# jiexray/gelly-streaming

Hardware: AMD Instinct MI355X
Metric: edges/sec (whole node) for streaming CC on RMAT-26 (higher is better)
Workload: dtype int64; 1 GPU; rmat26-cc-stream; scale=26, edges=1073741824, micro_batch=1048576, combine_every_edges_per_gpu=4194304, combine=none at 1 GPU (same cadence), ids=sparse 64-bit (scrambled), capacity_hint=33554432, vertices_labelled=32802821, parallelism=single GPU

## Files before the change

### gelly-streaming_amd/__init__.py

```python
import ctypes
import os

import numpy as np


_HERE = os.path.dirname(os.path.abspath(__file__))
LIB_PATH = os.path.join(_HERE, "lib", "libgs_summary.so")
if os.environ.get("GS_LIB_VARIANT"):
    LIB_PATH = os.path.join(_HERE, "lib_" + os.environ["GS_LIB_VARIANT"], "libgs_summary.so")

KIND_CC = 0
KIND_SIGNED = 1
KIND_DEGREE = 2

DEGREE_ALL = 0
DEGREE_IN = 1
DEGREE_OUT = 2

GS_OK = 0
GS_ERR_INVALID = -1
GS_ERR_HIP = -2
GS_ERR_CAPACITY = -3
GS_ERR_TRUNCATED = -4
GS_ERR_PARSE = -5
# ... 442 lines not shown


def digest_rows(v, label, parity=None):
    import torch

    def srl(x, k):
        return (x >> k) & ((1 << (64 - k)) - 1)

    def mix(z):
        z = (z ^ srl(z, 30)) * -4658895280553007687
        z = (z ^ srl(z, 27)) * -7723592293110705685
        return z ^ srl(z, 31)
    if v.numel() == 0:
        return 0
    a = mix(v ^ 0x243F6A8885A308D3)
    b = mix(label + (parity.to(torch.int64) * 0x13198A2E03707344 if parity is not None else 0))
    return int(torch.sum(a * b).item()) & ((1 << 64) - 1)


TESTING_KNOBS = {"server_idle_us": 0, "changes_walk_max": 1, "parse_lb_timeout_us": 2, "group_self_apply": 3,
                 "group_data_lag": 4, "degree_variant": 5, "triangle_variant": 6, "triangle_profile": 7,
                 "slice_profile": 8, "distinct_profile": 9, "spanner_round_cap": 10, "spanner_lds_set": 11,
                 "spanner_arenas": 12}


def testing_set(knob, value):
    _check(lib().gs_testing_set(TESTING_KNOBS[knob], -1 if value is None else int(value)))


def testing_get(knob):
    return lib().gs_testing_get(TESTING_KNOBS[knob])


def testing_hot_tune(summary, rows=None, sketch_log2=None, sample_folds=None):
    for what, v in enumerate((rows, sketch_log2, sample_folds)):
        if v is not None:
            _check(lib().gs_testing_hot_tune(summary._h, what, int(v)))


def testing_hot_keys(summary):
    import numpy as np
    n = lib().gs_testing_hot_keys(summary._h, None, 0)
    if n < 0:
        _check(int(n))
    out = (_i64 * max(int(n), 1))()
    m = lib().gs_testing_hot_keys(summary._h, out, int(n))
    if m < 0:
        _check(int(m))
    return np.frombuffer(out, dtype=np.int64, count=int(min(n, m))).copy()


class testing:

    def __init__(self, **knobs):
        self.knobs = knobs

    def __enter__(self):
        for k, v in self.knobs.items():
            testing_set(k, v)
        return self

    def __exit__(self, *a):
        for k in self.knobs:
            testing_set(k, None)


FAKE_COMM_PATH = os.path.join(_HERE, "host", "bin", "libgs_fakecomm.so")
_fake = None
# ... 1609 lines not shown
```

### gelly-streaming_amd/csrc/gs_capi.cpp

```cpp
#include <hip/hip_runtime.h>

#include <algorithm>
#include <atomic>
#include <chrono>
#include <mutex>
#include <unordered_map>
#include <cstdio>
#include <cstring>
#include <string>
#include <thread>
#include <vector>

#include "gs_ingest.h"
#include "gs_internal.hpp"

#ifndef GS_YOUNG_HEAD_LOG2
#define GS_YOUNG_HEAD_LOG2 14
#endif

namespace gsi {

thread_local std::string g_err;

int fail(int code, const std::string& msg) {
// ... 574 lines not shown

int fold_device_impl(gs_summary* h, const int64_t* src, const int64_t* dst, const uint8_t* w, size_t n,
                     size_t stride, size_t w_stride, bool track, bool check_cap, const FoldSource& fs) {
  if (n == 0) return GS_OK;
  const uint64_t units = fs.rows ? fs.units : n;
  if (track && !fs.take_out) {
    uint64_t fill = h->delta_fill_ub[h->dset];
    for (size_t off = 0; off < n; off += kMaxChunk) fill += per_shard_edges(std::min<size_t>(kMaxChunk, n - off));
    if (!h->drec || fill > h->delta_shard_cap)
      return fail(GS_ERR_CAPACITY, "delta list full: stage or take the delta records after at most " +
                                       std::to_string(h->delta_edges) + " folded edges");
  }
  constexpr int young_head_log2 = GS_YOUNG_HEAD_LOG2;
  const bool young_head = young_head_log2 > 0 && check_cap && !track && !fs.take_out && fs.lane < 0 && !fs.on_side &&
                          h->e_launched == 0 && h->nv_exact == 0 && n > ((size_t)2 << young_head_log2);
  if (check_cap && units) {
    if (int rc = ensure_capacity(h, units)) return rc;
  }
  const bool pipe = fs.allow_pipe && h->pipe_depth > 1 && (!track || fs.pipe_tracked) && fs.rows == 0 &&
                    !h->profiling && !h->changes;
  const bool on_lane = fs.lane >= 0 && !h->profiling;
  const bool side = fs.on_side && side_ok(h) && !track;
  if (!pipe && !side && !on_lane) {
    if (int rc = join_pipe_lanes(h)) return rc;
  }
  const bool sign = h->kind == GS_KIND_SIGNED;
  const int hot = (check_cap && !track && !fs.take_out && fs.rows == 0 && !fs.on_side && fs.lane < 0 && !fs.n_dev &&
                   stride != 3)
                      ? hot_log2(h)
                      : 0;
  for (size_t off = 0, c = 0; off < n; off += c) {
    const bool head = young_head && off == 0;
    c = head ? ((size_t)1 << young_head_log2) : std::min<size_t>(kMaxChunk, n - off);
    const uint32_t blocks = (uint32_t)((c + gs::kFoldBS - 1) / gs::kFoldBS);
    if (track && !fs.take_out) h->delta_fill_ub[h->dset] += per_shard_edges(c);
    hipStream_t st = side ? h->side : h->stream;
    if (side) h->side_dirty = true;
    if (head) {
      if (int rc = join_pipe_lanes(h)) return rc;
    } else if (pipe) {
      st = h->lane[h->lane_next];
      h->last_lane = h->lane_next;
      h->lane_next = (h->lane_next + 1) % h->pipe_depth;
      GS_HIP(hipEventRecord(h->main_ev, h->stream));
      if (hipEventQuery(h->main_ev) != hipSuccess) GS_HIP(hipStreamWaitEvent(st, h->main_ev, 0));
      h->lanes_dirty = true;
    } else if (on_lane) {
      st = h->lane[fs.lane];
      h->last_lane = fs.lane;
      h->lanes_dirty = true;
    }
    gs::FoldLaunch f;
    f.src = src + off * stride;
    f.dst = dst + off * stride;
    f.w = w ? w + off * w_stride : nullptr;
    f.n = c;
    f.stride = (uint32_t)stride;
    f.w_stride = (uint32_t)w_stride;
    if (h->dedup && !w && stride == 1 && fs.rows == 0 && !fs.n_dev) {
      int set = 0;
      if (st == h->side) set = gs_summary::kDedupSets - 1;
      for (int li = 0; li < gs_summary::kLanes; ++li)
        if (st == h->lane[li]) set = 1 + li;
      if (h->dd_edges[set] < c) {
        GS_HIP(hipStreamSynchronize(st));
        h->dd_edges[set] = 0;
        const uint64_t e = next_pow2(c);
        GS_HIP(h->dd_tab[set].alloc(2 * e * 2));
        GS_HIP(h->dd_w[set].alloc(e));
        h->dd_edges[set] = e;
      }
      const uint64_t slots = 2 * next_pow2(c);
      GS_HIP(hipMemsetAsync(h->dd_tab[set], 0xFF, slots * 16, st));
      GS_LAUNCH(gs::launch_dedup(f.src, f.dst, c, h->dd_tab[set], (uint32_t)(slots - 1), h->dd_w[set], st));
      f.w = h->dd_w[set];
      f.w_stride = 1;
    }
    f.rows = fs.rows;
    f.skip_rank = fs.skip_rank;
    f.counts = fs.counts;
    f.base = (uint32_t)off;
    f.n_dev = fs.n_dev;
    f.fail_in = off == 0 ? fs.fail_in : nullptr;
    f.shard0 = h->shard0;
    if (fs.take_out) {
      f.take_out = fs.take_out;
      f.take_cap = fs.take_cap;
      f.take_count = fs.take_count;
      f.done = h->done_dev;
      f.seq = *fs.take_seq = ++h->done_seq;
    }
    h->shard0 = (h->shard0 + blocks) & (gs::kShards - 1);
    const int rs = report_stream(h, st);
    const bool carry = check_cap && units && !fs.take_out && !fs.n_dev && h->rep_pending[rs];
    if (carry) {
      f.rep_out = h->rep.dev() + (h->rep_seq++ % gs_summary::kRepRing);
      f.rep_claim = h->rep_pending[rs];
      f.rep_epoch = (unsigned)(h->rep_epoch & 7u);
    }
    if (hot) {
      if (int rc = hot_before_fold(h)) return rc;
      if (h->hot_live >= 0 && h->hot_alloc_log2 == hot) {
        f.hot.e = h->hot_buf[h->hot_live];
        f.hot.shift = 65 - hot;
      }
    }
    {
      Prof p(h, KID_FOLD, st);
      gs::launch_fold(sign, track, h->table(), h->delta(), f, st);
    }
    GS_HIP(hipGetLastError());
    if (carry) {
      h->rep_pending_edges -= f.rep_claim;
      h->rep_pending[rs] = 0;
    }
    if (check_cap && units) {
      const uint64_t cu = fs.rows ? (off + c >= n ? units : 0) : c;
      h->rep_pending[rs] += cu;
      h->rep_pending_edges += cu;
      if (fs.n_dev && !fs.take_out)
        if (int rc = launch_report_now(h, rs, st)) return rc;
    }
    if (hot)
      if (int rc = hot_after_fold(h, f.src, f.dst, c, stride, st, hot)) return rc;
  }
  return GS_OK;
}

int join_into_last_lane(gs_summary* h, hipStream_t* es, bool* on_lane) {
  if (int rc = server_stop(h)) return rc;
  *es = h->stream;
  *on_lane = h->lanes_dirty && !h->side_dirty && h->last_lane >= 0 && h->lane[h->last_lane] && !h->profiling;
  if (!*on_lane) return join_lanes(h);
  *es = h->lane[h->last_lane];
  for (int i = 0; i < gs_summary::kLanes && h->lane[i]; ++i) {
    if (i == h->last_lane) continue;
    GS_HIP(hipEventRecord(h->lane[i].ev, h->lane[i]));
    GS_HIP(hipStreamWaitEvent(*es, h->lane[i].ev, 0));
  }
  GS_HIP(hipEventRecord(h->main_ev, h->stream));
  if (h->xwait || hipEventQuery(h->main_ev) != hipSuccess) GS_HIP(hipStreamWaitEvent(*es, h->main_ev, 0));
  return GS_OK;
// ... 1070 lines not shown
    h->hot_alloc_log2 = 0;
    for (auto& b : h->hot_buf) b.reset();
    h->hot_scratch.reset();
  }
  h->hot_cfg = log2_entries < 0 ? -1 : log2_entries;
  h->hot_first = first_after_edges;
  h->hot_every = rebuild_every_folds;
  return GS_OK;
}

int gs_hot_index_stats(gs_handle h, uint64_t* out4) {
  if (int rc = check_any(h)) return rc;
  if (!out4) return fail(GS_ERR_INVALID, "out is null");
  DeviceGuard g(h->device);
  if (int rc = join_lanes(h)) return rc;
  GS_HIP(hipStreamSynchronize(h->stream));
  if (int rc = hot_before_fold(h)) return rc;
  out4[0] = h->hot_builds;
  out4[1] = 0;
  out4[2] = h->hot_live >= 0 ? (uint64_t)h->hot_alloc_log2 : 0;
  out4[3] = h->hot_refreshes;
  if (h->hot_live >= 0) {
    std::vector<gs::HotBucket> e(gs::hot_buckets(h->hot_alloc_log2));
    GS_HIP(hipMemcpy(e.data(), h->hot_buf[h->hot_live], e.size() * sizeof(gs::HotBucket), hipMemcpyDeviceToHost));
    for (const gs::HotBucket& x : e) out4[1] += (x.key[0] != gs::kEmpty) + (x.key[1] != gs::kEmpty);
  }
  return GS_OK;
}

int gs_testing_hot_tune(void* hv, int what, int64_t value) {
  gs_handle h = static_cast<gs_handle>(hv);
  if (int rc = check_any(h)) return rc;
  if (h->kind != GS_KIND_CC) return fail(GS_ERR_INVALID, "the hot index serves connected-components summaries only");
  if (what < 0 || what > 2) return fail(GS_ERR_INVALID, "hot tune: what is 0, 1 or 2");
  if (value >= 0) {
    if (what == 0 && value != 1 && value != 2) return fail(GS_ERR_INVALID, "hot tune: 1 or 2 sketch rows");
    if (what == 1 && value > 6) return fail(GS_ERR_INVALID, "hot tune: at most 2^6 counters per id");
    if (what == 2 && value != 1 && value != 2 && value != 4) return fail(GS_ERR_INVALID, "hot tune: 1, 2 or 4 sample folds");
  }
  DeviceGuard g(h->device);
  if (int rc = join_lanes(h)) return rc;
  GS_HIP(hipStreamSynchronize(h->stream));
  hot_drop(h);
  h->hot_alloc_log2 = 0;
  for (auto& b : h->hot_buf) b.reset();
  h->hot_scratch.reset();
  if (what == 0) h->hot_rows = value < 0 ? 0 : (int)value;
  if (what == 1) h->hot_sketch_log2 = value < 0 ? -1 : (int)value;
  if (what == 2) h->hot_sample_folds = value < 0 ? 0u : (uint32_t)value;
  return GS_OK;
}

int64_t gs_testing_hot_keys(void* hv, int64_t* out, uint64_t cap) {
  gs_handle h = static_cast<gs_handle>(hv);
  if (int rc = check_any(h)) return rc;
  if (!out && cap) return fail(GS_ERR_INVALID, "out is null");
  DeviceGuard g(h->device);
  if (int rc = join_lanes(h)) return rc;
  GS_HIP(hipStreamSynchronize(h->stream));
  if (int rc = hot_before_fold(h)) return rc;
  if (h->hot_live < 0) return 0;
  std::vector<gs::HotBucket> e(gs::hot_buckets(h->hot_alloc_log2));
  GS_HIP(hipMemcpy(e.data(), h->hot_buf[h->hot_live], e.size() * sizeof(gs::HotBucket), hipMemcpyDeviceToHost));
  uint64_t n = 0;
  for (const gs::HotBucket& x : e)
    for (int64_t k : x.key)
      if (k != gs::kEmpty) {
// ... 58 lines not shown
```

### gelly-streaming_amd/csrc/gs_internal.hpp

```cpp
#pragma once
#include <hip/hip_runtime.h>

#include <string>
#include <vector>

#include "gs_devbuf.hpp"
#include "gs_grow.hpp"
#include "gs_hostio.hpp"
#include "gs_ingest.hpp"
#include "gs_kernels.hpp"
#include "gs_own.hpp"
#include "gs_sort.hpp"
#include "gs_summary.h"
#include "gs_testing.h"

namespace gsi {

int fail(int code, const std::string& msg);
int64_t testing_value(int knob, int64_t product);

constexpr int kMaxDevices = 64;
uint64_t create_capacity(uint64_t capacity_hint);
uint64_t create_bytes(uint64_t cap);

// ... 274 lines not shown
  uint64_t deg_total = 0;
  gsi::TextIngest text;
  int pipe_depth = 1;
  uint64_t api_calls = 0;
  int group_lanes = 0;
  static constexpr int kLanes = 4;
  gsi::Lane lane[kLanes];
  gsi::Event main_ev;
  gsi::Event idle_ev;
  bool xwait = false;
  int lane_next = 0;
  int last_lane = -1;
  bool lanes_dirty = false;
  bool export_ctr_zero = false;
  int hot_cfg = 0;
  uint64_t hot_first = 0;
  uint32_t hot_every = 0;
  gsi::DevBuf<gs::HotBucket> hot_buf[2];
  gsi::DevBuf<unsigned long long> hot_scratch;
  int hot_alloc_log2 = 0;
  int hot_live = -1;
  int hot_building = -1;
  gsi::Event hot_built;
  gsi::Event hot_read[2][kLanes + 1];
  bool hot_read_on[2] = {false, false};
  uint64_t hot_edges = 0;
  uint32_t hot_folds = 0;
  uint32_t hot_folds_r = 0;
  uint64_t hot_builds = 0;
  uint64_t hot_refreshes = 0;
  int hot_rows = 0, hot_sketch_log2 = -1;
  uint32_t hot_sample_folds = 0;
  uint32_t hot_counted = 0;
  gsi::Event hot_zeroed;
  gsi::Event hot_count_ev[3];
  hipStream_t side = nullptr;
  hipEvent_t side_ev = nullptr;
  bool side_dirty = false;
  bool dedup = false;
  static constexpr int kDedupSets = kLanes + 2;
  gsi::DevBuf<unsigned long long> dd_tab[kDedupSets];
  gsi::DevBuf<uint8_t> dd_w[kDedupSets];
  uint64_t dd_edges[kDedupSets] = {};
  uint64_t dd_kept_hint = 0;
  bool srv_on = false, srv_running = false;
  int srv_fits = -1;
  gsi::WindowServer srv;
  unsigned long long srv_seq = 0;
  uint64_t srv_launches = 0, srv_windows = 0;
  bool profiling = false;
  gsi::SpanTimer spans;
  uint64_t launches[gsi::KID_N] = {0, 0, 0, 0};
  double total_ms[gsi::KID_N] = {0, 0, 0, 0};

  gs::Table table() const {
    gs::Table t = gsi::make_table(tab, ctr, cap, logcap);
    t.vlist = vlist;
    t.vshard_cap = vshard_cap;
    t.mark_new = changes ? 1 : 0;
    t.hflags = h_flags.dev();
    return t;
  }
  gs::Delta delta(int set = -1) const {
    if (set < 0) set = dset;
    gs::Delta D;
    D.drec = drec ? drec + (size_t)set * gs::kShards * delta_shard_cap * 3 : nullptr;
// ... 58 lines not shown
```

### gelly-streaming_amd/csrc/gs_kernels.hip

```cpp
#include "gs_device.hpp"
#include "gs_kernels.hpp"

namespace gs {

__global__ __launch_bounds__(256) void k_init(Slot* tab, uint64_t nslots, uint32_t* ctr) {
  if (ctr && blockIdx.x == 0)
    for (uint32_t i = threadIdx.x; i < (uint32_t)CTR_COUNT; i += blockDim.x)
      *reinterpret_cast<uint4*>(ctr + ctr_index((int)i)) = make_uint4(0, 0, 0, 0);
  for (uint64_t s = (uint64_t)blockIdx.x * blockDim.x + threadIdx.x; s < nslots;
       s += (uint64_t)gridDim.x * blockDim.x) {
    uint4 v;
    v.x = 0u;
    v.y = 0x80000000u;
    v.z = (uint32_t)(s << 1);
    v.w = 0u;
    *reinterpret_cast<uint4*>(tab + s) = v;
  }
}

__device__ __forceinline__ uint64_t vlist_prefix(const Table& t, uint32_t* cnt, uint64_t* pre) {
  if (threadIdx.x < (uint32_t)kShards) cnt[threadIdx.x] = min(t.ctr[ctr_index(CTR_NV + threadIdx.x)], t.vshard_cap);
  __syncthreads();
  if (threadIdx.x == 0) {
    uint64_t o = 0;
// ... 81 lines not shown
  unsigned long long seq;
  bool server = false;
  unsigned long long* rep_out = nullptr;
  unsigned long long rep_claim = 0;
  unsigned rep_epoch = 0;
  HotIndex hot;
};

__device__ __forceinline__ void report_wave(uint32_t* ctr, unsigned long long n, unsigned long long* out,
                                            unsigned epoch) {
  unsigned long long done = 0;
  if (threadIdx.x == 0)
    done = atomicAdd(reinterpret_cast<unsigned long long*>(ctr + ctr_index(CTR_EDONE)), n) + n;
  done = __shfl(done, 0, 64);
  uint32_t c = threadIdx.x < (uint32_t)kShards
                   ? __hip_atomic_load(ctr + ctr_index(CTR_NV + threadIdx.x), __ATOMIC_RELAXED, __HIP_MEMORY_SCOPE_AGENT)
                   : 0u;
#pragma unroll
  for (int o = 32; o >= 1; o >>= 1) c += __shfl_xor(c, o, 64);
  if (threadIdx.x == 0) {
    const unsigned long long w = ((unsigned long long)c << 34) | ((unsigned long long)(epoch & 7u) << 31) |
                                 (done & ((1ull << 31) - 1));
    __hip_atomic_store(out, w, __ATOMIC_RELAXED, __HIP_MEMORY_SCOPE_SYSTEM);
  }
}

#ifndef GS_ROWS_TTAS
#define GS_ROWS_TTAS 3
#endif
#ifndef GS_COMBINE_ROUNDS
#define GS_COMBINE_ROUNDS 2
#endif
constexpr int kCombineRounds = GS_COMBINE_ROUNDS;

#ifdef GS_BLOCKLOG
struct BlockLog {
  unsigned long long t0, t1;
  unsigned long long src, tab;
  uint32_t blk, nblk, n, xcc;
  uint32_t hwid, valid, fresh, hooks;
};
__device__ BlockLog* g_blog = nullptr;
__device__ unsigned long long g_blog_cap = 0;
__device__ unsigned long long g_blog_n = 0;
#endif

#ifdef GS_SERVER_TRACE
__device__ unsigned long long* g_strace = nullptr;
__device__ unsigned long long g_strace_cap = 0;
#endif

#ifndef GS_TAKE_CARRY
#define GS_TAKE_CARRY 1
#endif
__device__ __forceinline__ unsigned long long tk_pack(unsigned long long n, unsigned long long rows,
                                                      unsigned long long newv) {
  return n | (rows << 16) | (newv << 40);
}
__device__ __forceinline__ unsigned long long tk_n(unsigned long long w) { return w & 0xFFFFull; }
__device__ __forceinline__ unsigned long long tk_rows(unsigned long long w) { return (w >> 16) & 0xFFFFFFull; }
__device__ __forceinline__ unsigned long long tk_newv(unsigned long long w) { return w >> 40; }

__device__ __forceinline__ bool take_tail(const Table& t, const FoldArgs& a, const int64_t* lrec, uint32_t lcnt,
                                          bool signed_kind, uint32_t blk, uint32_t nblocks, uint32_t newv = 0) {
  __shared__ unsigned long long base_sh;
  __shared__ uint32_t last_sh;
// ... 174 lines not shown
#else
  fold_block<SIGNED, TRACK, TAKE, ROWS, HOT>(t, D, a, blockIdx.x, failed, n_word, nullptr);
#endif
#ifdef GS_BLOCKLOG
  if (!SIGNED) {
    __syncthreads();
    if (threadIdx.x == 0 && g_blog) {
      const unsigned long long k = atomicAdd(&g_blog_n, 1ull);
      if (k < g_blog_cap) {
        BlockLog r;
        r.t0 = dbg_t0;
        r.t1 = wall_clock64();
        r.src = (unsigned long long)a.src;
        r.tab = (unsigned long long)t.tab;
        r.blk = blockIdx.x;
        r.nblk = gridDim.x;
        r.n = a.n;
        r.xcc = __builtin_amdgcn_s_getreg((3 << 11) | 20);
        r.hwid = __builtin_amdgcn_s_getreg((31 << 11) | 4);
        r.valid = dbg[0];
        r.fresh = dbg[1];
        r.hooks = dbg[2];
        g_blog[k] = r;
      }
    }
  }
#endif
  if (TAKE) {
    __syncthreads();
    take_tail(t, a, lrec, lcnt, SIGNED, blockIdx.x, gridDim.x);
  }
}

template <bool SIGNED, bool TRACK, bool TAKE, bool ROWS, bool HOT>
__device__ __forceinline__ void fold_block(const Table& t, const Delta& D, const FoldArgs& a, uint32_t blk,
                                           bool failed, unsigned long long n_word, uint32_t* dbg) {
  const int shard = (int)((blk + a.shard0) & (kShards - 1));
  const uint32_t i = blk * kFoldBS + threadIdx.x;
  bool valid = i < a.n && !failed;
  if (valid && a.n_dev) valid = (unsigned long long)(a.base + i) < (n_word & (kFailBit - 1));
  if (valid && a.rows) {
    const uint32_t ig = a.base + i, r = ig / a.rows, j = ig - r * a.rows;
    const unsigned long long cw = __hip_atomic_load(a.counts + r, __ATOMIC_RELAXED, __HIP_MEMORY_SCOPE_AGENT);
    if (SIGNED && j == 0 && (cw & kFailBit) && (int)r != a.skip_rank) atomicOr(&t.ctr[ctr_index(CTR_FAIL)], 1u);
    valid = (int)r != a.skip_rank && (unsigned long long)j < (cw & (kFailBit - 1));
  }
  const uint32_t wi = (valid && a.w) ? a.w[(size_t)i * a.w_stride] : 1u;
  if (wi & 0x80u) valid = false;
  const int64_t ks = valid ? __builtin_nontemporal_load(a.src + (size_t)i * a.stride) : 0;
  const int64_t kd = valid ? __builtin_nontemporal_load(a.dst + (size_t)i * a.stride) : 0;
  uint32_t need = SIGNED ? (wi & 1u) : 0u;
  const uint32_t hu = hash_slot(ks, t.shift), hv = hash_slot(kd, t.shift);
  int64_t k0u = 0, k0v = 0;
  uint32_t l0u = 0, l0v = 0;
  if (HOT) {
    static_assert(!HOT || (!SIGNED && !TRACK && !TAKE && !ROWS), "the hot index serves the plain CC fold only");
    const auto* hh = (const __attribute__((address_space(4))) HotHeader*)hot_header(a.hot);
    const uint32_t g = hh->g, g2 = hh->g2;
    bool hitu = false, hitv = false;
    if (valid) {
      hitu = hot_load(a.hot.e + hot_pos(ks, a.hot.shift), ks);
      hitv = hot_load(a.hot.e + hot_pos(kd, a.hot.shift), kd);
      if (!hitu) load_slot(t.tab + hu, k0u, l0u);
      if (!hitv) load_slot(t.tab + hv, k0v, l0v);
    }
    if (hitu || hitv) {
      const int64_t km = hitu ? kd : ks, k0m = hitu ? k0v : k0u;
      const uint32_t sm = hitu ? hv : hu, pm = (hitu ? l0v : l0u) >> 1;
      if ((hitu && hitv) || (k0m == km && km != kEmpty && (pm == g || pm == g2 || sm == g || sm == g2))) {
        GS_DBG(CTR_DBG_EDGES);
        GS_DBG(CTR_DBG_HOTHIT);
        valid = false;
      } else {
        GS_DBG(CTR_DBG_HOTFALL);
        if (hitu) load_slot(t.tab + hu, k0u, l0u);
        if (hitv) load_slot(t.tab + hv, k0v, l0v);
      }
    }
  } else if (valid) {
    load_slot(t.tab + hu, k0u, l0u);
    load_slot(t.tab + hv, k0v, l0v);
  }
  uint32_t ru = 0, rv = 0, lu = 0, lv = 0;
  int64_t kru = 0, krv = 0;
  bool act = false;
  NewVertices nvx;
  uint32_t fresh0 = kNoSlot, fresh1 = kNoSlot;
  bool has_rec = false;
  int64_t rec[3] = {0, 0, 0};
  bool nu = false, nv = false;
  uint32_t su = kNoSlot, sv = kNoSlot;
  if (valid) {
    GS_DBG(CTR_DBG_EDGES);
    constexpr bool kTu = !TAKE && (GS_INSERT_TTAS || TRACK || (ROWS && (GS_ROWS_TTAS & 1)));
    constexpr bool kTv = !TAKE && (GS_INSERT_TTAS || TRACK || (ROWS && (GS_ROWS_TTAS & 2)));
    if (GS_PAIR_INSERT && k0u == kEmpty && k0v == kEmpty && hu != hv && ks != kd && ks != kEmpty && kd != kEmpty) {
      insert_pair<kTu, kTv>(t, ks, hu, kd, hv, su, lu, nu, sv, lv, nv);
    } else {
      su = lookup_resolve<kTu>(t, ks, hu, k0u, l0u, lu, nu);
      sv = lookup_resolve<kTv>(t, kd, hv, k0v, l0v, lv, nv);
    }
  }
  nvx = reserve_new_vertices(t, shard, nu, su, nv, sv, TAKE ? D.lnv : nullptr);
  if (valid) {
    if (nu) fresh0 = su;
    if (nv) fresh1 = sv;
    if (dbg) atomicAdd(&dbg[1], (nu ? 1u : 0u) + ((nv && sv != su) ? 1u : 0u));
    if (TRACK && nu && su == sv) {
      has_rec = true;
      rec[0] = ks;
      rec[1] = ks;
      rec[2] = 0;
    }
    ru = su;
    rv = sv;
// ... 2 lines not shown
      if (pu == pv || pu == sv || pv == su) {
        GS_DBG(CTR_DBG_SHORT);
        if (SIGNED) {
          const uint32_t par = (pu == pv) ? ((lu ^ lv) & 1u) : (pu == sv ? (lu & 1u) : (lv & 1u));
          if ((need ^ par) & 1u) atomicOr(&t.ctr[ctr_index(CTR_FAIL)], 1u);
        }
      } else {
        uint32_t pru = 0, prv = 0;
        kru = ks;
        krv = kd;
        find_root2<false>(t, ru, lu, kru, pru, rv, lv, krv, prv);
        need ^= pru ^ prv;
        if (ru == rv) {
          GS_DBG(CTR_DBG_SAME);
          if (SIGNED && (need & 1u)) atomicOr(&t.ctr[ctr_index(CTR_FAIL)], 1u);
        } else {
          act = true;
        }
      }
    }
  }
  if (__popcll(__ballot(act)) >= 2) combine_hooks(act, ru, kru, rv, krv, need, kCombineRounds);
  if (act) has_rec = hook<SIGNED, TRACK>(t, ru, ru << 1, kru, rv, rv << 1, krv, need, fresh0, fresh1, rec);
  if (TRACK) {
    if (!TAKE && GS_WAVE_APPEND)
      append_record_wave(t, D, shard, has_rec, rec[0], rec[1], rec[2]);
    else if (has_rec)
      append_record<TAKE>(t, D, shard, rec[0], rec[1], rec[2]);
  }
  write_new_vertices(t, shard, nvx);
  if (dbg) {
    if (valid) atomicAdd(&dbg[0], 1u);
    if (act) atomicAdd(&dbg[2], 1u);
  }
}

template <bool SIGNED>
__global__ __launch_bounds__(kFoldBS) void k_window_server(Table t, Delta D, ServerBox* box, ServerBcast* bc,
                                                           unsigned long long* done, unsigned long long seq0,
                                                           unsigned long long idle_ticks) {
  __shared__ int64_t lrec[kFoldBS * 3];
  __shared__ uint32_t lcnt, lnv;
  __shared__ unsigned long long w[8];
#ifdef GS_TEST_LATE_WORKGROUP
  if (blockIdx.x == gridDim.x - 1) {
    const unsigned long long t0 = wall_clock64();
    while (wall_clock64() - t0 < 100ull * GS_TEST_LATE_WORKGROUP) __builtin_amdgcn_s_sleep(8);
  }
#endif
  D.lrec = lrec;
  D.lcnt = &lcnt;
  D.lnv = &lnv;
  if (blockIdx.x == 0 && threadIdx.x < 64) {
    unsigned long long c =
        __hip_atomic_load(t.ctr + ctr_index(CTR_NV + threadIdx.x), __ATOMIC_RELAXED, __HIP_MEMORY_SCOPE_AGENT);
#pragma unroll
    for (int o = 32; o >= 1; o >>= 1) c += __shfl_xor(c, o, 64);
    if (threadIdx.x == 0)
      __hip_atomic_store(reinterpret_cast<unsigned long long*>(t.ctr + ctr_index(CTR_SRV_NV)), c, __ATOMIC_RELAXED,
                         __HIP_MEMORY_SCOPE_AGENT);
    __builtin_amdgcn_s_waitcnt(0);
  }
  unsigned long long last = seq0;
  unsigned long long last_done = 0;
#ifdef GS_SERVER_TRACE
  __shared__ unsigned long long tseen, tbc;
// ... 455 lines not shown
  (void)hipDeviceSynchronize();
  (void)hipMemcpyFromSymbol(&n, HIP_SYMBOL(gs::g_blog_n), sizeof n);
  return n;
}
namespace gs {
#endif
#ifdef GS_SERVER_TRACE
}
extern "C" int gs_debug_server_trace(void* buf, unsigned long long cap) {
  unsigned long long* p = static_cast<unsigned long long*>(buf);
  if (hipMemcpyToSymbol(HIP_SYMBOL(gs::g_strace), &p, sizeof p) != hipSuccess ||
      hipMemcpyToSymbol(HIP_SYMBOL(gs::g_strace_cap), &cap, sizeof cap) != hipSuccess)
    return -2;
  return hipDeviceSynchronize() == hipSuccess ? 0 : -2;
}
namespace gs {
#endif
void launch_init(Slot* tab, uint64_t nslots, hipStream_t st, uint32_t* ctr) {
  const uint64_t blocks = (nslots + 255) / 256;
  const uint64_t want = nslots < (1ull << 26) ? (blocks + 15) / 16 : blocks;
  const unsigned g = (unsigned)(want < 1 ? 1 : (want < (1u << 22) ? want : (1u << 22)));
  hipLaunchKernelGGL(k_init, dim3(g), dim3(256), 0, st, tab, nslots, ctr);
}

static unsigned list_grid(uint64_t bound) {
  const uint64_t b = (bound + 255) / 256;
  return (unsigned)(b < 1 ? 1 : (b > 16384 ? 16384 : b));
}

void launch_reset_list(const Table& t, uint32_t* nxt, uint64_t bound, hipStream_t st) {
  hipLaunchKernelGGL(k_reset_list, dim3(list_grid(bound)), dim3(256), 0, st, t, nxt);
}

void launch_fold(bool sign, bool track, const Table& t, const Delta& D, const FoldLaunch& f, hipStream_t st) {
  FoldArgs a{f.src,       f.dst,    f.w,      f.n,       f.stride,   f.w_stride,  f.rows,
             f.skip_rank, f.counts, f.base,   f.n_dev,   f.fail_in,  f.shard0,    f.take_out,
             f.take_cap,  f.take_count, f.done, f.seq};
  a.rep_out = f.rep_out;
  a.rep_claim = f.rep_claim;
  a.rep_epoch = f.rep_epoch;
  a.hot = f.hot;
  const dim3 g((f.n + kFoldBS - 1) / kFoldBS), b(kFoldBS);
  if (f.take_out) {
    if (sign) hipLaunchKernelGGL((k_fold<true, true, true>), g, b, 0, st, t, D, a);
    else hipLaunchKernelGGL((k_fold<false, true, true>), g, b, 0, st, t, D, a);
    return;
  }
  if ((f.rows || f.stride == 3) && !track) {
    if (sign) hipLaunchKernelGGL((k_fold<true, false, false, true>), g, b, 0, st, t, D, a);
    else hipLaunchKernelGGL((k_fold<false, false, false, true>), g, b, 0, st, t, D, a);
    return;
  }
  if (!sign && !track && f.hot.e) {
    hipLaunchKernelGGL((k_fold<false, false, false, false, true>), g, b, 0, st, t, D, a);
    return;
  }
  if (!sign && !track) hipLaunchKernelGGL((k_fold<false, false, false>), g, b, 0, st, t, D, a);
  if (!sign && track) hipLaunchKernelGGL((k_fold<false, true, false>), g, b, 0, st, t, D, a);
  if (sign && !track) hipLaunchKernelGGL((k_fold<true, false, false>), g, b, 0, st, t, D, a);
  if (sign && track) hipLaunchKernelGGL((k_fold<true, true, false>), g, b, 0, st, t, D, a);
}

void launch_window_server(bool sign, const Table& t, const Delta& D, ServerBox* box, ServerBcast* bc,
                          unsigned long long* done, unsigned long long seq0, unsigned long long idle_ticks,
                          hipStream_t st) {
  if (sign)
    hipLaunchKernelGGL(k_window_server<true>, dim3(kServerBlocks), dim3(kFoldBS), 0, st, t, D, box, bc, done, seq0,
                       idle_ticks);
  else
    hipLaunchKernelGGL(k_window_server<false>, dim3(kServerBlocks), dim3(kFoldBS), 0, st, t, D, box, bc, done, seq0,
                       idle_ticks);
}

int window_server_resident_blocks(bool sign, int device) {
  int per_cu = 0, cus = 0;
  const hipError_t e = sign ? hipOccupancyMaxActiveBlocksPerMultiprocessor(&per_cu, k_window_server<true>, kFoldBS, 0)
                            : hipOccupancyMaxActiveBlocksPerMultiprocessor(&per_cu, k_window_server<false>, kFoldBS, 0);
  if (e != hipSuccess || hipDeviceGetAttribute(&cus, hipDeviceAttributeMultiprocessorCount, device) != hipSuccess)
    return 0;
  return per_cu * cus;
}

void launch_export(const Table& t, int64_t* ov, int64_t* ol, uint8_t* op, uint64_t cap_out, hipStream_t st, int part,
                   int nparts, bool by_list) {
  const uint64_t all = (uint64_t)t.r0 + 1;
  const uint64_t s0 = all * (uint64_t)part / (uint64_t)nparts, s1 = all * (uint64_t)(part + 1) / (uint64_t)nparts;
  const uint64_t tile = (uint64_t)kExportPer * kExportBS;
  const uint64_t tiles = (s1 - s0 + tile - 1) / tile;
  const uint64_t cap_blocks = 4096ull * 256 / kExportBS;
  const unsigned g = (unsigned)(tiles < cap_blocks ? (tiles ? tiles : 1) : cap_blocks);
  hipLaunchKernelGGL(k_export, dim3(g), dim3(kExportBS), 0, st, t, ov, ol, op, cap_out, s0, s1,
                     (by_list && nparts == 1) ? 1 : 0);
}
// ... 41 lines not shown
```

### gelly-streaming_amd/csrc/gs_kernels.hpp

```cpp
#pragma once
#include <hip/hip_runtime.h>
#include <stdint.h>

#include "gs_device.hpp"

namespace gs {

struct FoldLaunch {
  const int64_t* src = nullptr;
  const int64_t* dst = nullptr;
  const uint8_t* w = nullptr;
  uint32_t n = 0;
  uint32_t stride = 1;
  uint32_t w_stride = 1;
  uint32_t rows = 0;
  int skip_rank = -1;
  const unsigned long long* counts = nullptr;
  uint32_t base = 0;
  const unsigned long long* n_dev = nullptr;
  const uint32_t* fail_in = nullptr;
  uint32_t shard0 = 0;
  int64_t* take_out = nullptr;
  unsigned long long take_cap = 0;
  unsigned long long* take_count = nullptr;
  unsigned long long* done = nullptr;
  unsigned long long seq = 0;
  unsigned long long* rep_out = nullptr;
  unsigned long long rep_claim = 0;
  unsigned rep_epoch = 0;
  HotIndex hot;
};

constexpr uint32_t kServerBlocks = 256;
constexpr uint64_t kServerMaxEdges = (uint64_t)kServerBlocks * kFoldBS;
constexpr unsigned long long kServerStop = 1ull << 63;
constexpr unsigned long long kServerTagMask = (1ull << 48) - 1;
__host__ __device__ constexpr unsigned long long tag_word(unsigned long long seq, unsigned long long v) {
  return (seq & 0xFFFFull) << 48 | (v & kServerTagMask);
}
__host__ __device__ constexpr unsigned long long done_value(unsigned long long seq, unsigned long long v) {
  return (seq & 0xFFFFull) << 48 | ((v >> 62) & 1ull) << 47 | (v & ((1ull << 47) - 1));
}
__host__ __device__ constexpr unsigned long long done_decode(unsigned long long w) {
  return (w & ((1ull << 47) - 1)) | ((w >> 47) & 1ull) << 62;
}
struct alignas(64) ServerBox {
  unsigned long long seq;
  unsigned long long src, dst, n, rec, cap, cnt, done_seq;
  unsigned long long exited;
  unsigned long long taken;
  unsigned long long bc_init;
  unsigned long long pad[5];
};
struct alignas(64) ServerBcast {
  unsigned long long seq, src, dst, n, rec, cap, cnt, done_seq;
};
void launch_window_server(bool sign, const Table& t, const Delta& D, ServerBox* box, ServerBcast* bc,
                          unsigned long long* done, unsigned long long seq0, unsigned long long idle_ticks,
                          hipStream_t st);
int window_server_resident_blocks(bool sign, int device);

void launch_init(Slot* tab, uint64_t nslots, hipStream_t st, uint32_t* ctr = nullptr);
void launch_dedup(const int64_t* src, const int64_t* dst, uint32_t n, unsigned long long* tab, uint32_t mask,
                  uint8_t* w, hipStream_t st);
void launch_reset_list(const Table& t, uint32_t* nxt, uint64_t bound, hipStream_t st);
void launch_fold(bool sign, bool track, const Table& t, const Delta& D, const FoldLaunch& f, hipStream_t st);
void launch_export(const Table& t, int64_t* ov, int64_t* ol, uint8_t* op, uint64_t cap_out, hipStream_t st,
                   int part = 0, int nparts = 1, bool by_list = false);
void launch_export_list(const Table& t, int64_t* ov, int64_t* ol, uint8_t* op, uint64_t cap_out, uint64_t bound,
                        hipStream_t st);
void launch_digest(const Table& t, unsigned long long* out, uint64_t bound, hipStream_t st);
void launch_stage(const Table& t, const Delta& D, int64_t* out, uint64_t cap, int width,
                  unsigned long long* count_out, bool with_fail, hipStream_t st);
void launch_report(uint32_t* ctr, uint64_t n, unsigned long long* out, unsigned epoch, hipStream_t st);
void launch_headers(const unsigned long long* counts, int nranks, long long* out, long long seq, hipStream_t st);
constexpr unsigned long long kSignalFlagBit = 1ull << 62;
void launch_signal(unsigned long long* out, unsigned long long seq, const uint32_t* vals, int nvals, int stride,
                   hipStream_t st, bool clear = false, const uint32_t* flag = nullptr);
void launch_find_one(const Table& t, int64_t key, int64_t* out, hipStream_t st);
void launch_find_batch(const Table& t, const int64_t* v, uint64_t n, int64_t* label, uint8_t* found, uint8_t* parity,
                       hipStream_t st);

struct HotTune {
  int rows;
  int sketch_log2;
};
inline uint64_t hot_buckets(int log2_ids) { return 1ull << (log2_ids - 1); }
uint64_t hot_scratch_words(int log2_ids, const HotTune& tune);
void launch_hot_zero(int log2_ids, const HotTune& tune, unsigned long long* scratch, hipStream_t st);
void launch_hot_count(const int64_t* src, const int64_t* dst, uint32_t n, uint32_t stride, int log2_ids,
                      const HotTune& tune, unsigned long long* scratch, hipStream_t st);
void launch_hot_build(const Table& t, const int64_t* src, const int64_t* dst, uint32_t n, uint32_t stride,
                      HotBucket* out, int log2_ids, const HotTune& tune, unsigned long long* scratch, hipStream_t st);
void launch_hot_refresh(const Table& t, HotBucket* live, int log2_ids, hipStream_t st);

void launch_iota(uint32_t* nxt, uint64_t n, hipStream_t st);
void launch_relist(const Table& t, uint32_t* nxt, hipStream_t st);
void launch_emit_records(const Table& t, uint32_t* nxt, const int64_t* rec, const unsigned long long* nrec,
                         uint64_t nrec_bound, uint32_t walk_max, int64_t* ov, int64_t* ol, uint8_t* op, uint64_t cap,
// ... 8 lines not shown
```

Measured before the change: 30.89 billion edges/s.

## Add tiled hot-index fold kernel that compacts unsettled edges into an LDS queue

Adds a k_fold_tile kernel for the CC hot-index fold path. Each wave settles edges through the hot index and a first slot probe, then ballots the edges that are still unresolved into a shared-memory queue. The block then runs the full union tail over the compacted queue, so lanes stay busy instead of diverging on mostly-settled waves. Defaults are K=1 with the queue on, so the new kernel replaces the old hot fold. This adds a __syncthreads, LDS traffic and a second slot load for queued edges, and shard advancement now follows the actual launched grid.

```diff
diff --git a/gelly-streaming_amd/__init__.py b/gelly-streaming_amd/__init__.py
--- a/gelly-streaming_amd/__init__.py
+++ b/gelly-streaming_amd/__init__.py
@@ -498,8 +498,8 @@
     return lib().gs_testing_get(TESTING_KNOBS[knob])
 
 
-def testing_hot_tune(summary, rows=None, sketch_log2=None, sample_folds=None):
-    for what, v in enumerate((rows, sketch_log2, sample_folds)):
+def testing_hot_tune(summary, rows=None, sketch_log2=None, sample_folds=None, tile_k=None, tile_queue=None):
+    for what, v in enumerate((rows, sketch_log2, sample_folds, tile_k, tile_queue)):
         if v is not None:
             _check(lib().gs_testing_hot_tune(summary._h, what, int(v)))
 
diff --git a/gelly-streaming_amd/csrc/gs_capi.cpp b/gelly-streaming_amd/csrc/gs_capi.cpp
--- a/gelly-streaming_amd/csrc/gs_capi.cpp
+++ b/gelly-streaming_amd/csrc/gs_capi.cpp
@@ -630,7 +630,6 @@
   for (size_t off = 0, c = 0; off < n; off += c) {
     const bool head = young_head && off == 0;
     c = head ? ((size_t)1 << young_head_log2) : std::min<size_t>(kMaxChunk, n - off);
-    const uint32_t blocks = (uint32_t)((c + gs::kFoldBS - 1) / gs::kFoldBS);
     if (track && !fs.take_out) h->delta_fill_ub[h->dset] += per_shard_edges(c);
     hipStream_t st = side ? h->side : h->stream;
     if (side) h->side_dirty = true;
@@ -688,7 +687,6 @@
       f.done = h->done_dev;
       f.seq = *fs.take_seq = ++h->done_seq;
     }
-    h->shard0 = (h->shard0 + blocks) & (gs::kShards - 1);
     const int rs = report_stream(h, st);
     const bool carry = check_cap && units && !fs.take_out && !fs.n_dev && h->rep_pending[rs];
     if (carry) {
@@ -701,11 +699,13 @@
       if (h->hot_live >= 0 && h->hot_alloc_log2 == hot) {
         f.hot.e = h->hot_buf[h->hot_live];
         f.hot.shift = 65 - hot;
+        f.hot_tile_k = h->hot_tile_k;
+        f.hot_tile_queue = h->hot_tile_queue;
       }
     }
     {
       Prof p(h, KID_FOLD, st);
-      gs::launch_fold(sign, track, h->table(), h->delta(), f, st);
+      h->shard0 = (h->shard0 + gs::launch_fold(sign, track, h->table(), h->delta(), f, st)) & (gs::kShards - 1);
     }
     GS_HIP(hipGetLastError());
     if (carry) {
@@ -1842,7 +1842,14 @@
   gs_handle h = static_cast<gs_handle>(hv);
   if (int rc = check_any(h)) return rc;
   if (h->kind != GS_KIND_CC) return fail(GS_ERR_INVALID, "the hot index serves connected-components summaries only");
-  if (what < 0 || what > 2) return fail(GS_ERR_INVALID, "hot tune: what is 0, 1 or 2");
+  if (what < 0 || what > 4) return fail(GS_ERR_INVALID, "hot tune: what is 0 .. 4");
+  if (what >= 3) {
+    if (what == 3 && value >= 0 && value != 1 && value != 2 && value != 4)
+      return fail(GS_ERR_INVALID, "hot tune: a tile of 1, 2 or 4 x 256 edges");
+    if (what == 3) h->hot_tile_k = value < 0 ? 0 : (int)value;
+    if (what == 4) h->hot_tile_queue = value < 0 ? -1 : (value != 0);
+    return GS_OK;
+  }
   if (value >= 0) {
     if (what == 0 && value != 1 && value != 2) return fail(GS_ERR_INVALID, "hot tune: 1 or 2 sketch rows");
     if (what == 1 && value > 6) return fail(GS_ERR_INVALID, "hot tune: at most 2^6 counters per id");
diff --git a/gelly-streaming_amd/csrc/gs_internal.hpp b/gelly-streaming_amd/csrc/gs_internal.hpp
--- a/gelly-streaming_amd/csrc/gs_internal.hpp
+++ b/gelly-streaming_amd/csrc/gs_internal.hpp
@@ -330,6 +330,7 @@
   int hot_rows = 0, hot_sketch_log2 = -1;
   uint32_t hot_sample_folds = 0;
   uint32_t hot_counted = 0;
+  int hot_tile_k = 0, hot_tile_queue = -1;
   gsi::Event hot_zeroed;
   gsi::Event hot_count_ev[3];
   hipStream_t side = nullptr;
diff --git a/gelly-streaming_amd/csrc/gs_kernels.hip b/gelly-streaming_amd/csrc/gs_kernels.hip
--- a/gelly-streaming_amd/csrc/gs_kernels.hip
+++ b/gelly-streaming_amd/csrc/gs_kernels.hip
@@ -137,6 +137,15 @@
 #define GS_COMBINE_ROUNDS 2
 #endif
 constexpr int kCombineRounds = GS_COMBINE_ROUNDS;
+#ifndef GS_HOT_TILE_K
+#define GS_HOT_TILE_K 1
+#endif
+#ifndef GS_HOT_TILE_QUEUE
+#define GS_HOT_TILE_QUEUE 1
+#endif
+static_assert(GS_HOT_TILE_K == 1 || GS_HOT_TILE_K == 2 || GS_HOT_TILE_K == 4, "GS_HOT_TILE_K");
+constexpr int kHotTileK = GS_HOT_TILE_K;
+constexpr bool kHotTileQueue = GS_HOT_TILE_QUEUE != 0;
 
 #ifdef GS_BLOCKLOG
 struct BlockLog {
@@ -377,11 +386,9 @@
   }
 }
 
-template <bool SIGNED, bool TRACK, bool TAKE, bool ROWS, bool HOT>
-__device__ __forceinline__ void fold_block(const Table& t, const Delta& D, const FoldArgs& a, uint32_t blk,
-                                           bool failed, unsigned long long n_word, uint32_t* dbg) {
-  const int shard = (int)((blk + a.shard0) & (kShards - 1));
-  const uint32_t i = blk * kFoldBS + threadIdx.x;
+template <bool SIGNED>
+__device__ __forceinline__ bool edge_valid(const Table& t, const FoldArgs& a, uint32_t i, bool failed,
+                                           unsigned long long n_word, uint32_t& wi) {
   bool valid = i < a.n && !failed;
   if (valid && a.n_dev) valid = (unsigned long long)(a.base + i) < (n_word & (kFailBit - 1));
   if (valid && a.rows) {
@@ -390,11 +397,33 @@
     if (SIGNED && j == 0 && (cw & kFailBit) && (int)r != a.skip_rank) atomicOr(&t.ctr[ctr_index(CTR_FAIL)], 1u);
     valid = (int)r != a.skip_rank && (unsigned long long)j < (cw & (kFailBit - 1));
   }
-  const uint32_t wi = (valid && a.w) ? a.w[(size_t)i * a.w_stride] : 1u;
+  wi = (valid && a.w) ? a.w[(size_t)i * a.w_stride] : 1u;
   if (wi & 0x80u) valid = false;
-  const int64_t ks = valid ? __builtin_nontemporal_load(a.src + (size_t)i * a.stride) : 0;
-  const int64_t kd = valid ? __builtin_nontemporal_load(a.dst + (size_t)i * a.stride) : 0;
-  uint32_t need = SIGNED ? (wi & 1u) : 0u;
+  return valid;
+}
+
+__device__ __forceinline__ int64_t edge_id(const int64_t* ids, const FoldArgs& a, uint32_t i, bool valid) {
+  return valid ? __builtin_nontemporal_load(ids + (size_t)i * a.stride) : 0;
+}
+
+__device__ __forceinline__ bool hot_one_hit_settles(int64_t km, uint32_t sm, int64_t k0m, uint32_t l0m, uint32_t g,
+                                                    uint32_t g2) {
+  const uint32_t pm = l0m >> 1;
+  return k0m == km && km != kEmpty && (pm == g || pm == g2 || sm == g || sm == g2);
+}
+
+template <bool SIGNED, bool TRACK, bool TAKE, bool ROWS>
+__device__ __forceinline__ void fold_tail(const Table& t, const Delta& D, const FoldArgs& a, int shard, bool valid,
+                                          int64_t ks, int64_t kd, uint32_t need, uint32_t hu, uint32_t hv, int64_t k0u,
+                                          uint32_t l0u, int64_t k0v, uint32_t l0v, uint32_t* dbg);
+
+template <bool SIGNED, bool TRACK, bool TAKE, bool ROWS, bool HOT>
+__device__ __forceinline__ void fold_edge(const Table& t, const Delta& D, const FoldArgs& a, int shard, uint32_t i,
+                                          bool failed, unsigned long long n_word, uint32_t* dbg) {
+  uint32_t wi;
+  bool valid = edge_valid<SIGNED>(t, a, i, failed, n_word, wi);
+  const int64_t ks = edge_id(a.src, a, i, valid), kd = edge_id(a.dst, a, i, valid);
+  const uint32_t need = SIGNED ? (wi & 1u) : 0u;
   const uint32_t hu = hash_slot(ks, t.shift), hv = hash_slot(kd, t.shift);
   int64_t k0u = 0, k0v = 0;
   uint32_t l0u = 0, l0v = 0;
@@ -411,8 +440,8 @@
     }
     if (hitu || hitv) {
       const int64_t km = hitu ? kd : ks, k0m = hitu ? k0v : k0u;
-      const uint32_t sm = hitu ? hv : hu, pm = (hitu ? l0v : l0u) >> 1;
-      if ((hitu && hitv) || (k0m == km && km != kEmpty && (pm == g || pm == g2 || sm == g || sm == g2))) {
+      const uint32_t sm = hitu ? hv : hu, l0m = hitu ? l0v : l0u;
+      if ((hitu && hitv) || hot_one_hit_settles(km, sm, k0m, l0m, g, g2)) {
         GS_DBG(CTR_DBG_EDGES);
         GS_DBG(CTR_DBG_HOTHIT);
         valid = false;
@@ -426,6 +455,20 @@
     load_slot(t.tab + hu, k0u, l0u);
     load_slot(t.tab + hv, k0v, l0v);
   }
+  fold_tail<SIGNED, TRACK, TAKE, ROWS>(t, D, a, shard, valid, ks, kd, need, hu, hv, k0u, l0u, k0v, l0v, dbg);
+}
+
+template <bool SIGNED, bool TRACK, bool TAKE, bool ROWS, bool HOT>
+__device__ __forceinline__ void fold_block(const Table& t, const Delta& D, const FoldArgs& a, uint32_t blk,
+                                           bool failed, unsigned long long n_word, uint32_t* dbg) {
+  fold_edge<SIGNED, TRACK, TAKE, ROWS, HOT>(t, D, a, (int)((blk + a.shard0) & (kShards - 1)),
+                                            blk * kFoldBS + threadIdx.x, failed, n_word, dbg);
+}
+
+template <bool SIGNED, bool TRACK, bool TAKE, bool ROWS>
+__device__ __forceinline__ void fold_tail(const Table& t, const Delta& D, const FoldArgs& a, int shard, bool valid,
+                                          int64_t ks, int64_t kd, uint32_t need, uint32_t hu, uint32_t hv, int64_t k0u,
+                                          uint32_t l0u, int64_t k0v, uint32_t l0v, uint32_t* dbg) {
   uint32_t ru = 0, rv = 0, lu = 0, lv = 0;
   int64_t kru = 0, krv = 0;
   bool act = false;
@@ -494,6 +537,106 @@
   if (dbg) {
     if (valid) atomicAdd(&dbg[0], 1u);
     if (act) atomicAdd(&dbg[2], 1u);
+  }
+}
+
+struct alignas(16) TileEdge {
+  int64_t s, d;
+};
+
+template <int K, bool QUEUE>
+__global__ __launch_bounds__(kFoldBS) __attribute__((amdgpu_waves_per_eu(8, 8))) void k_fold_tile(Table t, Delta D, FoldArgs a) {
+  static_assert(K == 1 || K == 2 || K == 4, "tile rounds");
+  if (a.rep_out && blockIdx.x == 0 && threadIdx.x < 64) report_wave(t.ctr, a.rep_claim, a.rep_out, a.rep_epoch);
+  const int shard = (int)((blockIdx.x + a.shard0) & (kShards - 1));
+  const uint32_t tile = blockIdx.x * (K * kFoldBS) + threadIdx.x;
+  if (!QUEUE) {
+    for (int r = 0; r < K; ++r)
+      fold_edge<false, false, false, false, true>(t, D, a, shard, tile + r * kFoldBS, false, 0ull, nullptr);
+    return;
+  }
+  __shared__ TileEdge queue[QUEUE ? K * kFoldBS : 1];
+  __shared__ uint32_t qfill[kFoldBS / 64];
+  const auto* hh = (const __attribute__((address_space(4))) HotHeader*)hot_header(a.hot);
+  const uint32_t g = hh->g, g2 = hh->g2;
+  int64_t ks[K], kd[K], k0u[K], k0v[K];
+  uint32_t l0u[K], l0v[K];
+  bool valid[K], hitu[K], hitv[K];
+#pragma unroll
+  for (int r = 0; r < K; ++r) {
+    uint32_t wi;
+    valid[r] = edge_valid<false>(t, a, tile + r * kFoldBS, false, 0ull, wi);
+    ks[r] = edge_id(a.src, a, tile + r * kFoldBS, valid[r]);
+    kd[r] = edge_id(a.dst, a, tile + r * kFoldBS, valid[r]);
+  }
+#pragma unroll
+  for (int r = 0; r < K; ++r) {
+    hitu[r] = hitv[r] = false;
+    if (valid[r]) {
+      hitu[r] = hot_load(a.hot.e + hot_pos(ks[r], a.hot.shift), ks[r]);
+      hitv[r] = hot_load(a.hot.e + hot_pos(kd[r], a.hot.shift), kd[r]);
+    }
+  }
+#pragma unroll
+  for (int r = 0; r < K; ++r) {
+    k0u[r] = k0v[r] = 0;
+    l0u[r] = l0v[r] = 0;
+    if (valid[r] && !hitu[r]) load_slot(t.tab + hash_slot(ks[r], t.shift), k0u[r], l0u[r]);
+    if (valid[r] && !hitv[r]) load_slot(t.tab + hash_slot(kd[r], t.shift), k0v[r], l0v[r]);
+  }
+  const uint32_t lane = threadIdx.x & 63u, wave = threadIdx.x >> 6;
+  TileEdge* mine = queue + wave * (K * 64);
+  uint32_t fill = 0;
+#pragma unroll
+  for (int r = 0; r < K; ++r) {
+    const uint32_t hu = hash_slot(ks[r], t.shift), hv = hash_slot(kd[r], t.shift);
+    bool done;
+    if (hitu[r] || hitv[r]) {
+      done = (hitu[r] && hitv[r]) || (hitu[r] ? hot_one_hit_settles(kd[r], hv, k0v[r], l0v[r], g, g2)
+                                              : hot_one_hit_settles(ks[r], hu, k0u[r], l0u[r], g, g2));
+      if (done) GS_DBG(CTR_DBG_HOTHIT);
+      else GS_DBG(CTR_DBG_HOTFALL);
+    } else {
+      const uint32_t pu = l0u[r] >> 1, pv = l0v[r] >> 1;
+      done = k0u[r] == ks[r] && k0v[r] == kd[r] && ks[r] != kEmpty && kd[r] != kEmpty &&
+             (hu == hv || pu == pv || pu == hv || pv == hu);
+      if (valid[r] && done && hu != hv) GS_DBG(CTR_DBG_SHORT);
+    }
+    if (valid[r] && done) GS_DBG(CTR_DBG_EDGES);
+    const bool put = valid[r] && !done;
+    const unsigned long long b = __ballot(put);
+    if (put) mine[fill + __builtin_amdgcn_mbcnt_hi((uint32_t)(b >> 32), __builtin_amdgcn_mbcnt_lo((uint32_t)b, 0u))] =
+                 TileEdge{ks[r], kd[r]};
+    fill += (uint32_t)__popcll(b);
+  }
+  if (lane == 0) qfill[wave] = fill;
+  __syncthreads();
+  uint32_t start[kFoldBS / 64 + 1];
+  start[0] = 0;
+#pragma unroll
+  for (int w = 0; w < (int)(kFoldBS / 64); ++w) start[w + 1] = start[w] + qfill[w];
+  const uint32_t len = start[kFoldBS / 64];
+  for (uint32_t q0 = 0; q0 < len; q0 += kFoldBS) {
+    const uint32_t q = q0 + threadIdx.x;
+    const bool v = q < len;
+    int64_t s = 0, d = 0;
+    if (v) {
+      uint32_t at = q;
+#pragma unroll
+      for (int x = 1; x < (int)(kFoldBS / 64); ++x)
+        if (q >= start[x]) at = x * (K * 64) + (q - start[x]);
+      const TileEdge e = queue[at];
+      s = e.s;
+      d = e.d;
+    }
+    const uint32_t hu = hash_slot(s, t.shift), hv = hash_slot(d, t.shift);
+    int64_t c0u = 0, c0v = 0;
+    uint32_t m0u = 0, m0v = 0;
+    if (v) {
+      load_slot(t.tab + hu, c0u, m0u);
+      load_slot(t.tab + hv, c0v, m0v);
+    }
+    fold_tail<false, false, false, false>(t, D, a, shard, v, s, d, 0u, hu, hv, c0u, m0u, c0v, m0v, nullptr);
   }
 }
 
@@ -1015,7 +1158,7 @@
   hipLaunchKernelGGL(k_reset_list, dim3(list_grid(bound)), dim3(256), 0, st, t, nxt);
 }
 
-void launch_fold(bool sign, bool track, const Table& t, const Delta& D, const FoldLaunch& f, hipStream_t st) {
+uint32_t launch_fold(bool sign, bool track, const Table& t, const Delta& D, const FoldLaunch& f, hipStream_t st) {
   FoldArgs a{f.src,       f.dst,    f.w,      f.n,       f.stride,   f.w_stride,  f.rows,
              f.skip_rank, f.counts, f.base,   f.n_dev,   f.fail_in,  f.shard0,    f.take_out,
              f.take_cap,  f.take_count, f.done, f.seq};
@@ -1027,21 +1170,30 @@
   if (f.take_out) {
     if (sign) hipLaunchKernelGGL((k_fold<true, true, true>), g, b, 0, st, t, D, a);
     else hipLaunchKernelGGL((k_fold<false, true, true>), g, b, 0, st, t, D, a);
-    return;
+    return g.x;
   }
   if ((f.rows || f.stride == 3) && !track) {
     if (sign) hipLaunchKernelGGL((k_fold<true, false, false, true>), g, b, 0, st, t, D, a);
     else hipLaunchKernelGGL((k_fold<false, false, false, true>), g, b, 0, st, t, D, a);
-    return;
+    return g.x;
   }
   if (!sign && !track && f.hot.e) {
-    hipLaunchKernelGGL((k_fold<false, false, false, false, true>), g, b, 0, st, t, D, a);
-    return;
+    const int k = f.hot_tile_k ? f.hot_tile_k : kHotTileK;
+    const bool queue = f.hot_tile_queue < 0 ? kHotTileQueue : f.hot_tile_queue != 0;
+    const dim3 gt((f.n + k * kFoldBS - 1) / (k * kFoldBS));
+    if (k == 1 && !queue) hipLaunchKernelGGL((k_fold<false, false, false, false, true>), g, b, 0, st, t, D, a);
+    else if (k == 1) hipLaunchKernelGGL((k_fold_tile<1, true>), gt, b, 0, st, t, D, a);
+    else if (k == 2 && queue) hipLaunchKernelGGL((k_fold_tile<2, true>), gt, b, 0, st, t, D, a);
+    else if (k == 2) hipLaunchKernelGGL((k_fold_tile<2, false>), gt, b, 0, st, t, D, a);
+    else if (queue) hipLaunchKernelGGL((k_fold_tile<4, true>), gt, b, 0, st, t, D, a);
+    else hipLaunchKernelGGL((k_fold_tile<4, false>), gt, b, 0, st, t, D, a);
+    return gt.x;
   }
   if (!sign && !track) hipLaunchKernelGGL((k_fold<false, false, false>), g, b, 0, st, t, D, a);
   if (!sign && track) hipLaunchKernelGGL((k_fold<false, true, false>), g, b, 0, st, t, D, a);
   if (sign && !track) hipLaunchKernelGGL((k_fold<true, false, false>), g, b, 0, st, t, D, a);
   if (sign && track) hipLaunchKernelGGL((k_fold<true, true, false>), g, b, 0, st, t, D, a);
+  return g.x;
 }
 
 void launch_window_server(bool sign, const Table& t, const Delta& D, ServerBox* box, ServerBcast* bc,
diff --git a/gelly-streaming_amd/csrc/gs_kernels.hpp b/gelly-streaming_amd/csrc/gs_kernels.hpp
--- a/gelly-streaming_amd/csrc/gs_kernels.hpp
+++ b/gelly-streaming_amd/csrc/gs_kernels.hpp
@@ -29,6 +29,7 @@
   unsigned long long rep_claim = 0;
   unsigned rep_epoch = 0;
   HotIndex hot;
+  int hot_tile_k = 0, hot_tile_queue = -1;
 };
 
 constexpr uint32_t kServerBlocks = 256;
@@ -64,7 +65,7 @@
 void launch_dedup(const int64_t* src, const int64_t* dst, uint32_t n, unsigned long long* tab, uint32_t mask,
                   uint8_t* w, hipStream_t st);
 void launch_reset_list(const Table& t, uint32_t* nxt, uint64_t bound, hipStream_t st);
-void launch_fold(bool sign, bool track, const Table& t, const Delta& D, const FoldLaunch& f, hipStream_t st);
+uint32_t launch_fold(bool sign, bool track, const Table& t, const Delta& D, const FoldLaunch& f, hipStream_t st);
 void launch_export(const Table& t, int64_t* ov, int64_t* ol, uint8_t* op, uint64_t cap_out, hipStream_t st,
                    int part = 0, int nparts = 1, bool by_list = false);
 void launch_export_list(const Table& t, int64_t* ov, int64_t* ol, uint8_t* op, uint64_t cap_out, uint64_t bound,
```

New measurement: 31.11 billion edges/s (median of 6 runs). Within noise of the previous version (+0.7%).
